# sleveque/control

Measured on AMD Instinct MI355X. Metric: Krylov iterations/s (preconditioned GMRES(10), all-at-once heat-control KKT), higher is better.
Workload: dtype f64; 1 GPU; 2-D heat control, 256^2 P1, n_t=64, beta=0.0001, T=2, BE, mode G; unknowns=8454272, krylov=gmres, left preconditioning, restart 10, classical Gram-Schmidt, parallelism=time-block rows over 1 GPU(s), transport=none, sweep_tiles=boxes from the dof coordinates (kkt_set_tile_coordinates)

## Files before the change

control_amd/csrc/capi.cpp:

```cpp
#include <algorithm>
#include <charconv>
#include <climits>
#include <cmath>
#include <cstring>
#include <string>

#include "comm.hpp"
#include "pc.hpp"
#include "relin.hpp"
#include "system.hpp"
#include "tiles.hpp"

using namespace kkt;

struct kkt_system {
    System S;
};

static std::string g_create_error;

#define KKT_TRY(h, ...)                                   \
    if (!(h)) return KKT_ERR_ARG;                         \
    System &S = (h)->S;                                   \
    try {                                                 \
// ... 15 lines not shown
    o.*F = v[0] == '1';
    return true;
}
template <int Options::*F, int LO = INT_MIN, int HI = INT_MAX>
static bool set_int(Options &o, const char *v) {
    int x = 0;
    const auto r = std::from_chars(v, v + std::strlen(v), x);
    if (r.ec != std::errc() || *r.ptr || x < LO || x > HI) return false;
    o.*F = x;
    return true;
}
static bool set_prog_mode(Options &o, const char *v) {
    static const char *names[] = {"auto", "tile", "dataflow", "flags", "w"};
    for (int k = 0; k < 5; ++k)
        if (std::strcmp(v, names[k]) == 0) {
            o.prog_mode = (ProgMode)k;
            return true;
        }
    return false;
}
static bool set_coarse_setup(Options &o, const char *v) {
    o.coarse_columns = std::strcmp(v, "columns") == 0;
    return o.coarse_columns || std::strcmp(v, "batched") == 0;
}

struct OptionKey {
    const char *key, *accepted;
    bool (*set)(Options &, const char *);
};
static const OptionKey option_keys[] = {
    {"sell_r", "1 | 2", set_int<&Options::sell_r, 1, 2>},
    {"sell_sort", "0 | 1", set_switch<&Options::sell_sort>},
    {"sell_sigma", "1..64", set_int<&Options::sell_sigma, 1, 64>},
    {"shared_rows", "0 | 1", set_switch<&Options::shared_rows>},
    {"ragged_switch", "0 | 1", set_switch<&Options::ragged_switch>},
    {"ragged_xcd", "0 | 1", set_switch<&Options::ragged_xcd>},
    {"apply_xcd", "0 | 1", set_switch<&Options::apply_xcd>},
    {"pc_xcd", "0 | 1", set_switch<&Options::pc_xcd>},
    {"interleave", "0 | 1", set_switch<&Options::interleave>},
    {"kernarg_ops", "0 | 1", set_switch<&Options::kernarg_ops>},
    {"no_graph", "0 | 1", set_switch<&Options::no_graph>},
    {"persistent", "0 | 1", set_switch<&Options::persistent>},
    {"prog_mode", "auto | tile | dataflow | flags | w", set_prog_mode},
    {"prog_waves", "1..8", set_int<&Options::prog_waves, 1, 8>},
    {"prog_steps", "0 | 1", set_switch<&Options::prog_steps>},
    {"tile_depth", "1..16", set_int<&Options::tile_depth, 1, TILE_MAX_DEPTH>},
    {"tile_waves", "1..16", set_int<&Options::tile_waves, 1, 16>},
    {"tile_unfused", "0 | 1", set_switch<&Options::tile_unfused>},
    {"tile_poll_delay", "an integer", set_int<&Options::tile_poll_delay>},
    {"lanes", "0 | 1", set_switch<&Options::lanes>},
    {"lane_chunks", "an integer", set_int<&Options::lane_chunks>},
    {"coarse_setup", "batched | columns", set_coarse_setup},
    {"coarse_keep", "0 | 1", set_switch<&Options::coarse_keep>},
    {"coarse_blocks", "0 | 1", set_switch<&Options::coarse_blocks>},
    {"coarse_rings", "0 | 1", set_switch<&Options::coarse_rings>},
    {"stage_timers", "0 | 1", set_switch<&Options::stage_timers>},
    {"verbose", "0 | 1", set_switch<&Options::verbose>},
    {"stamps", "0 | 1", set_switch<&Options::stamps>},
    {"debug_drop_handoff", "an integer", set_int<&Options::debug_drop_handoff>},
};

extern "C" {

int kkt_create(kkt_handle *out, int device_id) {
    if (!out) return KKT_ERR_ARG;
    *out = nullptr;
    try {
        int ndev = 0;
        if (hipGetDeviceCount(&ndev) != hipSuccess || ndev < 1)
            fail(KKT_ERR_HIP, "no HIP device available: libkkt has no CPU path");
        if (device_id < 0 || device_id >= ndev) fail(KKT_ERR_ARG, "device id out of range");
        HIPCHK(hipSetDevice(device_id));
        auto h = std::make_unique<kkt_system>();
        h->S.device = device_id;
        h->S.own_stream = Stream::create();
        h->S.stream = h->S.own_stream;
        *out = h.release();
        return KKT_OK;
// ... 496 lines not shown
```

control_amd/csrc/kernels.hpp:

```cpp
#pragma once
#include <hip/hip_runtime_api.h>
#include <stdint.h>

#include <string>

namespace kkt {

struct TileLaunchError {
    std::string msg;
};

constexpr int MAX_TERMS = 8;
constexpr int MDOT_MAX = 8;
constexpr int REDUCE_BLOCKS = 1024;

struct VRef {
    int64_t off;
    int32_t base;
    int32_t pad_;
};
struct Bases { const double *p[4]; };

struct SpmvTerm {
    const double *vals;
// ... 140 lines not shown
    int32_t fused_update;
    int32_t hslots;
};
bool tile_sweep_available(int W, int rpt, int threads, int hslots);
bool tile_sweep_coarse_available(int W, int rpt, int threads, int hslots);
int tile_sweep_max_hslots(int W, int rpt, int threads);
int tile_sweep_max_rpt(int W, int threads);
bool tile_sweep_fuses_update(int W, int max_terms);
size_t tile_sweep_lds_bytes(int nk_pad, int its, int coarse_nc = 0, int coarse_nslots = 0,
                            int coarse_jmax = 0, int coarse_nr_max = 0,
                            int coarse_einv_rows = 0,
                            int coarse_einv_width = 0,
                            int coarse_ring_entries = 0,
                            int coarse_jxmax = 0);
size_t tile_sweep_lds_bytes(int nk_pad, int its, const TileCoarseDev &c, int cache, bool rings);
size_t tile_sweep_lds_bytes(int nk_pad, int its, const TileCoarseDev &c);
int tile_sweep_max_tiles(int W, int rpt, int threads, size_t lds_bytes, int hslots,
                         bool coarse = false);
void launch_tile_sweep(hipStream_t s, const TileArgs &a, const TileLevel *d_levels,
                       const int32_t *d_n, const int32_t *d_grow, const uint16_t *d_lcol,
                       const int32_t *d_gpos, const uint8_t *d_rowmask, int ntiles, int threads,
                       size_t granule_words, const TileCoarseDev *h_coarse = nullptr);

void launch_csr_to_sell(hipStream_t s, const double *csr_vals, const int32_t *sell2csr,
                        double *sell_vals, int64_t n_padded);
void launch_mask_columns(hipStream_t s, double *sell_vals, const int32_t *col,
                         const uint8_t *colmask, int64_t n_padded);
void launch_vals_axpy(hipStream_t s, double *out, const double *a, double c,
                      const double *b, int64_t n_padded);
void launch_vals_differ(hipStream_t s, const double *a, const double *b, int64_t n, unsigned *flag);
void launch_vals_sym_skew(hipStream_t s, const double *a, const int32_t *tpos, double *h,
                          double *sk, int64_t n, unsigned *nonsym);
void launch_extract_dinv(hipStream_t s, const int32_t *col, const int32_t *slice_off,
                         const double *vals, const uint8_t *rowmask, double *dinv,
                         int nrows, int nslices, int R, const int32_t *perm = nullptr);

void launch_copy(hipStream_t s, double *y, const double *x, int64_t n);
void launch_fill(hipStream_t s, double *y, double v, int64_t n);
void launch_axpby(hipStream_t s, double *y, double a, const double *x, double b, int64_t n);
struct MaskJob { const uint8_t *mask; double alpha; };
void launch_mask_blocks(hipStream_t s, double *y, const double *x, const double *mx,
                        const MaskJob *d_jobs, int nblocks, int64_t nx);
void launch_time_transform_mask(hipStream_t s, double *y, const double *t, const double *xin,
                                const MaskJob *d_jobs, int kind, int n, int64_t nx,
                                const double *lo_halo, const double *hi_halo);
void launch_time_transform(hipStream_t s, double *y, const double *x, int kind, int n,
// ... 63 lines not shown
```

control_amd/csrc/pc.cpp:

```cpp
#include "pc.hpp"

#include <algorithm>
#include <chrono>
#include <cmath>
#include <cstdlib>
#include <cstdio>
#include <cstring>

namespace kkt {

static VRef vabs(const double *p) {
    return p ? VRef{(int64_t)(uintptr_t)p, 0, 0} : VRef{0, -1, 0};
}

SchurPC::SchurPC(System &S, const kkt_pc_desc &d) : S_(S), d_(d) {
    if (!S.finalized) fail(KKT_ERR_STATE, "kkt_set_pc_schur needs a finalized system");
    if (d.kind < KKT_PC_STATIONARY || d.kind > KKT_PC_INSTATIONARY_CN)
        fail(KKT_ERR_ARG, "unknown preconditioner kind");
    if (!d.m_indptr || !d.m_indices || !d.m_values) fail(KKT_ERR_ARG, "mass matrix missing");
    if (S.nx0 != S.nx1 || d.nx != S.nx0)
        fail(KKT_ERR_ARG, "built-in preconditioner needs equal spatial spaces of size nx");
    nx_ = d.nx;
    if (d.kind == KKT_PC_STATIONARY)
        n_ = 1;
// ... 23 lines not shown
        if (p_indptr_[0] != 0 || pn < 0) fail(KKT_ERR_ARG, "bad P indptr");
        p_indices_.assign(d.p_indices, d.p_indices + pn);
        p_values_.assign(d.p_values, d.p_values + pn);
        for (int64_t r = 0; r < nx_; ++r)
            if (p_indptr_[r + 1] < p_indptr_[r]) fail(KKT_ERR_ARG, "P indptr not monotone");
        for (int32_t c : p_indices_)
            if (c < 0 || c >= d.n_coarse) fail(KKT_ERR_ARG, "P column index out of range");
    }
    d_.p_indptr = d_.p_indices = nullptr;
    d_.p_values = nullptr;
    d_.m_indptr = d_.m_indices = nullptr;
    d_.m_values = nullptr;
    d_.bc_idx = nullptr;
    use_graph_ = !S_.opts.no_graph;
    use_programs_ = S_.opts.persistent;
    use_lanes_ = S_.opts.lanes;
    build();
}

void SchurPC::clear_program() {
    segments_.clear();
    program_mem_.release();
    il_cap_ = 0;
    sweep_levels_.clear();
    steps_.clear();
    n_events_ = 0;
    cur_lane_ = 0;
}

int SchurPC::emit_record(int lane) {
    PcStep s;
    s.kind = PcStep::EV_RECORD;
    s.lane = lane;
    s.ev = n_events_++;
    steps_.push_back(s);
    return s.ev;
}

void SchurPC::emit_wait(int lane, int ev) {
    PcStep s;
    s.kind = PcStep::EV_WAIT;
    s.lane = lane;
    s.ev = ev;
    steps_.push_back(s);
}

// ... 437 lines not shown
    if (coarse && !tile_sweep_fuses_update(tile_plan_.W, max_terms)) return false;
    if (tile_sweep_fuses_update(tile_plan_.W, max_terms) &&
        !(tile_plan_.W > 9 && S_.opts.tile_unfused && !coarse)) {
        tile_step(levels.data(), (int)levels.size(), (int)(e - k), true);
        return true;
    }
    for (size_t i = 0; i < run.size(); ++i) {
        const SweepLevel &lv = *run[i];
        TileLevel L = levels[i];
        size_t first_cheb = lv.first;
        if (L.n_upd > 0) {
            out.push_back(steps_[lv.first]);
            first_cheb = lv.first + 1;
            L.n_upd = 0;
            L.prev_in_lds = 0;
            L.bin = lv.b_after;
            L.bout = nullptr;
        }
        tile_step(&L, 1, (int)(lv.last - first_cheb), false);
    }
    return true;
}

void SchurPC::fuse_programs() {
    if (!use_programs_) return;
    if (!d_err_) {
        d_err_ = handle_mem_.alloc<unsigned>(64 + 16 * 1024);
        HIPCHK(hipMemset(d_err_, 0, (64 + 16 * 1024) * sizeof(unsigned)));
    }
    const bool tile_wanted = S_.opts.prog_mode == ProgMode::Auto || S_.opts.prog_mode == ProgMode::Tile;
    const bool use_tiles = tile_wanted && prepare_tiles();
    tile_epoch_cursor_ = 0;
    tile_cepoch_cursor_ = 0;
    tile_cleared_ = false;
    if (!legacy_tried_) {
        legacy_tried_ = true;
        legacy_ok_ = setup_row_programs();
    }
    if (!use_tiles && !legacy_ok_) {
        use_programs_ = false;
        return;
    }
    auto gather_out = [](const RowOp &op) -> int64_t {
        return (op.mode == EPI_LIN && op.y2.base >= 0) ? op.y2.off : op.y.off;
    };
    std::vector<PcStep> out;
    auto emit_prog = [&](size_t q0, size_t q1) {
        std::vector<RowOp> ops;
// ... 93 lines not shown
        if (s.kind == PcStep::PROG && form < 3) form = std::max(form, s.granule ? 2 : 1);
    }
    S_.info.sweep_form = form;
    S_.info.sweep_tiles = form == 3 ? tile_plan_.ntiles : 0;
    S_.info.sweep_threads = form == 3 ? tile_plan_.threads : 0;
    S_.info.sweep_depth = form == 3 ? tile_plan_.depth : 0;
    S_.info.sweep_row_slots = form == 3 ? tile_plan_.rpt : 0;
    bool rings = false;
    for (const PcStep &s : steps_)
        if (s.kind == PcStep::TILE && s.coarse) rings = h_tile_coarse_.ring_prolong != 0;
    S_.info.sweep_coarse_rings = rings ? 1 : 0;
}

void SchurPC::plain_forms(std::vector<int32_t> &out) const {
    const Pattern &P = S_.patterns[m_pat_];
    for (const PcStep &s : steps_) {
        if (s.kind == PcStep::ROWS) {
            const int form = s.rows.shared_matrix && s.rows.R == 2 ? KKT_PC_ROWS_SHARED
                             : s.rows.single                       ? KKT_PC_ROWS_KERNARG
                                                                   : KKT_PC_ROWS_PLAIN;
            out.insert(out.end(), {form, s.rows.uniform_w, s.rows.R, s.lane, s.rows.nops, 0});
        } else if (s.kind == PcStep::ROWS_IL) {
            out.insert(out.end(), {KKT_PC_ROWS_INTERLEAVED, s.il_w, 2, s.lane, s.il_groups, 0});
        } else if (s.kind == PcStep::PROG) {
            out.insert(out.end(), {KKT_PC_PROGRAM, P.uniform_w, P.R, s.lane, s.nphases,
                                   s.gmode == 2 ? 2 : s.granule ? 1 : 0});
        } else if (s.kind == PcStep::TILE) {
            out.insert(out.end(), {KKT_PC_TILE, tile_plan_.W, tile_plan_.rpt, s.lane,
                                   tile_plan_.threads, (s.fused ? 1 : 0) | (s.coarse ? 2 : 0)});
        }
    }
}

void SchurPC::debug_read(unsigned long long *out, int n) {
    if (!d_err_) return;
    HIPCHK(hipStreamSynchronize(S_.stream));
    HIPCHK(hipMemcpy(out, d_err_ + 64, (size_t)n * 8, hipMemcpyDeviceToHost));
    HIPCHK(hipMemset(d_err_ + 64, 0, (size_t)n * 8));
}

void SchurPC::time_programs(float *ms, int *launches, int64_t *phases) {
    hipStream_t st = S_.stream;
    *ms = 0.f;
    *launches = 0;
    *phases = 0;
    std::vector<std::pair<Event, Event>> evs;
// ... 33 lines not shown
    for (size_t k = 0; k < steps_.size(); ++k) {
        replay(k, k + 1);
        HIPCHK(hipEventRecord(ev[k + 1], st));
    }
    HIPCHK(hipStreamSynchronize(st));
    for (size_t k = 0; k < steps_.size(); ++k) {
        float ms = 0.f;
        HIPCHK(hipEventElapsedTime(&ms, ev[k], ev[k + 1]));
        const PcStep &s = steps_[k];
        out->total_ms += ms;
        if (s.kind == PcStep::PROG || s.kind == PcStep::TILE) {
            out->sweeps_ms += ms;
            out->sweep_launches += 1;
            out->sweep_phases += s.nphases;
        } else if (s.kind == PcStep::ROWS && s.rows.nops == 1 && n_ > 1) {
            out->sweeps_ms += ms;
            out->sweep_launches += 1;
            out->sweep_phases += 1;
        } else if (s.kind == PcStep::COMM) {
            out->comm_ms += ms;
            out->comm_steps += 1;
        } else {
            out->batched_ms += ms;
            if (s.kind == PcStep::ROWS || s.kind == PcStep::TIME || s.kind == PcStep::ROWS_IL)
                out->batched_launches += 1;
        }
    }
}

bool SchurPC::timed_out(std::string *why) {
    if (!d_err_) return false;
    unsigned e = 0;
    HIPCHK(hipMemcpyAsync(&e, d_err_, sizeof e, hipMemcpyDeviceToHost, S_.stream));
    HIPCHK(hipStreamSynchronize(S_.stream));
    if (!e) return false;
    unsigned rec[40] = {0};
    HIPCHK(hipMemcpy(rec, d_err_, sizeof rec, hipMemcpyDeviceToHost));
    HIPCHK(hipMemset(d_err_, 0, sizeof rec));
    std::string msg = "persistent sweep kernel timed out waiting for a neighbour workgroup";
    if (e & 4u)
        msg += " (tile form: tile " + std::to_string(rec[8]) + ", hand-off " +
               std::to_string(rec[9]) + ", local row " + std::to_string(rec[10]) +
               ", global row " + std::to_string(rec[11]) + ", tags seen new " +
               std::to_string(rec[12]) + "/" + std::to_string(rec[13]) + " old " +
               std::to_string(rec[14]) + "/" + std::to_string(rec[15]) +
               (rec[16] ? ", both iterates)" : ", newest iterate only)");
    if (e & 8u)
// ... 809 lines not shown
bool SchurPC::emit_solves_interleaved(const std::vector<Solve> &sv, int its, double emin,
                                      double emax) {
    if (!S_.opts.interleave || S_.opts.lanes) return false;
    const size_t m = sv.size();
    for (const Solve &q : sv)
        if (q.vals != sv[0].vals || q.dinv != sv[0].dinv) return false;
    const Pattern &P = S_.patterns[m_pat_];
    if (P.R != 2) return false;
    const int ng = (int)((m + 3) / 4);
    const size_t need = (size_t)ng * 4 * (size_t)nx_;
    if (need > il_cap_) {
        for (int k = 0; k < 3; ++k) {
            il_P_[k] = program_mem_.alloc<double>(need + 32);
            HIPCHK(hipMemsetAsync(il_P_[k], 0, (need + 32) * sizeof(double), S_.stream));
        }
        il_cap_ = need;
    }
    const double scale = 2.0 / (emax + emin);
    const double alpha = 1.0 - scale * emin, mu = 1.0 / alpha, omegaprod = 2.0 / alpha;
    double c_km1 = 1.0, c_k = mu;
    auto buf = [&](int step, int g) -> double * {
        return il_P_[(step - 1) % 3] + (size_t)g * 4 * (size_t)nx_;
    };
    for (int step = 1; step <= its; ++step) {
        double k1 = 0.0, k2 = 0.0, k3 = scale;
        if (step >= 2) {
            const double c_kp1 = 2.0 * mu * c_k - c_km1;
            const double omega = omegaprod * c_k / c_kp1;
            k1 = 1.0 - omega;
            k2 = omega;
            k3 = scale * omega;
            c_km1 = c_k;
            c_k = c_kp1;
        }
        const bool last = step == its;
        std::vector<IlOp> ops(ng);
        for (int g = 0; g < ng; ++g) {
            IlOp op{};
            op.col = P.d_col;
            op.slice_off = P.d_slice_off;
            op.perm = P.d_perm;
            op.vals = sv[0].vals;
            op.dinv = sv[0].dinv;
            op.rowmask = mask_;
            op.nrows = (int32_t)nx_;
            op.nslices = P.nslices;
            op.uniform_w = P.uniform_w;
            op.nlev = (int32_t)std::min<size_t>(4, m - (size_t)g * 4);
            for (int l = 0; l < op.nlev; ++l) {
                op.b[l] = sv[(size_t)g * 4 + l].b;
                op.out[l] = last ? sv[(size_t)g * 4 + l].out : nullptr;
            }
            op.x = step >= 2 ? buf(step - 1, g) : nullptr;
            op.pkm1 = step >= 3 ? buf(step - 2, g) : nullptr;
            op.y = last ? nullptr : buf(step, g);
            op.c1 = k1;
            op.c2 = k2;
            op.c3 = k3;
            for (int l = 0; l < 4; ++l) {
                const bool live = last && l < op.nlev;
                op.post1[l] = live ? sv[(size_t)g * 4 + l].post1 : 1.0;
                op.post2[l] = live ? sv[(size_t)g * 4 + l].post2 : 1.0;
            }
            ops[g] = op;
        }
        PcStep s;
        s.kind = PcStep::ROWS_IL;
        s.d_il = program_mem_.upload(ops.data(), ops.size());
        s.il_groups = ng;
        s.il_slices = P.nslices;
        s.il_w = P.uniform_w;
        s.lane = cur_lane_;
        steps_.push_back(s);
    }
    return true;
}

void SchurPC::emit_solves(const std::vector<Solve> &sv, int its, double emin, double emax,
                          double *const P[3], int64_t pstride, bool first_done,
                          std::vector<TileCoef> *coef_out, double eimag, const Mat *mat) {
    if (coarse_cycles_ > 0 && mat && mat->einv && sv.size() == 1 && !first_done) {
        emit_coarse_solve(nullptr, sv[0], *mat);
        return;
    }
    const size_t m = sv.size();
    if (m >= 4 && !first_done && its >= 2 && eimag == 0.0 && pstride == nx_ &&
        emit_solves_interleaved(sv, its, emin, emax))
        return;
    SweepLevel solo;
    const bool record_solo = m == 1 && !first_done && its >= 2;
    if (record_solo) {
        solo.first = steps_.size();
        coef_out = &solo.coef;
    }
    std::vector<Cheb> ops(m);
    if (its == 0) {
        for (size_t q = 0; q < m; ++q)
// ... 296 lines not shown
    if (n_events_ > 0 && !side_) side_ = Stream::create();
    while ((int)events_.size() < n_events_) events_.push_back(Event::create(false));
    for (size_t k = first; k < last; ++k) {
        const PcStep &s = steps_[k];
        hipStream_t st = s.lane == 0 ? S_.stream : side_;
        switch (s.kind) {
            case PcStep::EV_RECORD:
                HIPCHK(hipEventRecord(events_[s.ev], st));
                break;
            case PcStep::EV_WAIT:
                HIPCHK(hipStreamWaitEvent(st, events_[s.ev], 0));
                break;
            case PcStep::ROWS:
                if (s.rows.shared_matrix &&
                    launch_rowops_shared(st, s.rows.d_ops, s.rows.nops, s.rows.max_slices,
                                         s.rows.R, s.rows.uniform_w, xcd))
                    break;
                launch_rowops(st, s.rows.d_ops, s.rows.nops, s.rows.max_slices, s.rows.R, B, 1,
                              s.rows.uniform_w, s.rows.single ? &s.rows.h_op : nullptr);
                break;
            case PcStep::ROWS_IL:
                launch_rowops_il(st, s.d_il, s.il_groups, s.il_slices, s.il_w, xcd);
                break;
            case PcStep::TIME:
                launch_time_transform(st, s.y, s.x, s.tkind, s.n, s.nx, s.lo_halo, s.hi_halo);
                break;
            case PcStep::COPY:
                launch_copy(st, s.y, s.x, s.nx);
                break;
            case PcStep::COARSE:
                launch_coarse_correction(st, coarse_, s.einv, s.cr, s.x, s.y, s.nx);
                break;
            case PcStep::PROG: {
                const Pattern &P = S_.patterns[m_pat_];
                if (s.gmode == 2)
                    launch_row_program_gw(st, s.rows.d_ops, s.nphases, prog_nwg_, prog_wpw_, d_g0_,
                                          d_g1_, granule_words_, d_err_);
                else if (s.granule)
                    launch_row_program_g(st, s.rows.d_ops, s.d_lite, s.nphases, prog_nwg_, prog_wpw_,
                                         P.uniform_w, d_g0_, d_g1_, granule_words_, d_err_);
                else
                    launch_row_program(st, s.rows.d_ops, s.nphases, prog_nwg_, prog_wpw_, P.R,
                                       P.uniform_w, d_dep_, d_flags_, d_err_, prog_lowreg_);
                break;
            }
            case PcStep::TILE: {
// ... 73 lines not shown
```

control_amd/csrc/pc.hpp:

```cpp
#pragma once
#include <map>
#include <string>
#include <vector>

#include "comm.hpp"
#include "system.hpp"
#include "tiles.hpp"

namespace kkt {

struct Spectrum {
    double emin, emax;
    int steps;
};
Spectrum jacobi_spectrum(System &S, int pattern, const double *vals, const double *dinv,
                         const uint8_t *rowmask, int max_steps,
                         bool zero_mean = false);
double jacobi_skew_radius(System &S, int pattern, const double *skew_vals, const double *dinv,
                          const uint8_t *rowmask, int max_steps, int *steps_out);

struct PcStep {
    enum Kind { ROWS, TIME, COPY, COMM, PROG, TILE, EV_RECORD, EV_WAIT, COARSE, ROWS_IL } kind;
    IlOp *d_il = nullptr;
    int il_groups = 0, il_slices = 0, il_w = 0;
    const double *einv = nullptr;
    const double *cr = nullptr;
    int lane = 0;
    int ev = -1;
    RowLaunch rows;
    double *y = nullptr;
    const double *x = nullptr;
    int tkind = 0, n = 0;
    int64_t nx = 0;
    const double *lo_halo = nullptr, *hi_halo = nullptr;
    int dst = -1, src = -1;
    int nphases = 0;
    bool granule = false;
    PhaseLite *d_lite = nullptr;
    int gmode = 0;
    TileLevel *d_levels = nullptr;
    int nlevels = 0, its = 0;
    uint32_t epoch0 = 0;
    bool fused = true;
    bool clear = false;
    bool coarse = false;
// ... 182 lines not shown
    struct Cheb {
        const double *vals;
        const double *dinv, *b, *pk, *pkm1;
        double *y;
        double c1, c2, c3, post1 = 1.0, post2 = 1.0;
    };
    void build();
    void clear_program();
    const double *block_vals(int q, int i, int j) const;
    Mat schur_matrix(const double *base_vals, double c, bool solved = true);
    void emit_lin(const std::vector<Lin> &ops);
    void emit_cheb(const std::vector<Cheb> &ops);
    double *il_P_[3] = {nullptr, nullptr, nullptr};
    size_t il_cap_ = 0;
    void emit_time(double *y, const double *x, int kind, int n, const double *lo_halo = nullptr,
                   const double *hi_halo = nullptr);
    void emit_comm(const double *send, int dst, double *recv, int src);
    struct Solve {
        const double *vals, *dinv, *b;
        double *out;
        double post1 = 1.0, post2 = 1.0;
    };
    bool emit_solves_interleaved(const std::vector<Solve> &sv, int its, double emin, double emax);
    void emit_solves(const std::vector<Solve> &sv, int its, double emin, double emax,
                     double *const P[3], int64_t pstride, bool first_done = false,
                     std::vector<TileCoef> *coef_out = nullptr, double eimag = 0.0,
                     const Mat *mat = nullptr);
    void emit_update_and_solve(Lin upd, const Solve &sv, int its, double emin, double emax,
                               double eimag = 0.0, const Mat *mat = nullptr);
    void emit_coarse_solve(const Lin *upd, const Solve &sv, const Mat &F);
    const int32_t *transpose_positions();
    int32_t *d_tpos_ = nullptr;
    bool tpos_tried_ = false;
    void push_rows(std::vector<RowOp> &r);
    void build_stationary();
    void build_BE();
    void build_CN();
    void replay(size_t first, size_t last);
};

class StokesPC : public PcBase {
   public:
    StokesPC(System &outer, System &inner, System &commutator, const kkt_pc_stokes_desc &d);
    void run() override;
    double *in() override { return in_; }
    double *out() override { return out_; }
// ... 48 lines not shown
```

control_amd/csrc/system.hpp:

```cpp
#pragma once
#include <hip/hip_runtime_api.h>
#include <stdint.h>

#include <map>
#include <memory>
#include <string>
#include <tuple>
#include <vector>

#include "../../include/kkt.h"
#include "devmem.hpp"
#include "kernels.hpp"

namespace kkt {

struct Error {
    int code;
    std::string msg;
};
[[noreturn]] void fail(int code, const std::string &msg);
enum class ProgMode { Auto, Tile, Dataflow, Flags, W };
struct Options {
    int sell_r = 2, sell_sigma = 8;
    bool sell_sort = true, shared_rows = true, ragged_switch = true;
    bool ragged_xcd = true, apply_xcd = false, pc_xcd = true;
    bool interleave = true, kernarg_ops = false, no_graph = false, lanes = false;
    int lane_chunks = 4;
    bool persistent = true, prog_steps = true, tile_unfused = false;
    ProgMode prog_mode = ProgMode::Auto;
    int prog_waves = 0, tile_depth = 0, tile_waves = 0;
    bool coarse_columns = false;
    bool coarse_keep = false, coarse_blocks = true;
    bool coarse_rings = true;
    bool stage_timers = false, verbose = false, stamps = false;
    int tile_poll_delay = 24, debug_drop_handoff = 0;
};

struct Pattern {
    int64_t nrows = 0, ncols = 0, nnz = 0;
    int R = 2;
    int nslices = 0;
    int64_t nslots = 0;
    int64_t npadded = 0;
    int max_width = 0;
    int uniform_w = -1;
    uint64_t hash = 0;
    std::vector<int32_t> h_indptr, h_indices;
    int32_t *d_col = nullptr;
    int32_t *d_slice_off = nullptr;
    std::vector<int32_t> h_slice_off;
    int64_t sell_index(int64_t r, int k) const {
        const int64_t C = 64 * R, pos = pos_of(r), s = pos / C, rin = pos - s * C;
        return ((int64_t)h_slice_off[s] + k) * C + (rin % 64) * R + rin / 64;
    }
    int32_t *d_sell2csr = nullptr;
    std::vector<int32_t> h_row_of, h_pos_of;
// ... 223 lines not shown
```

control_amd/multiblock.py:

```python
from __future__ import annotations

import ctypes as C
import os
from dataclasses import dataclass
from typing import Optional, Sequence

import numpy as np

from . import _lib

__all__ = ["Nullspace", "NoneNullspace", "ConstantNullspace", "DirichletBCNullspace",
           "FullNullspace", "MultiBlockSystem", "SchurPC", "StokesPC", "KSPResult",
           "ChebSpec", "PatternOnly"]

Q00, Q01, Q10, Q11 = 0, 1, 2, 3
_KSP_TYPES = {"gmres": 0, "fgmres": 1, "minres": 2}
_PC_SIDES = {"left": 0, "right": 1, 0: 0, 1: 1}


class Nullspace:
    """``preconditioner.py:75-116`` (the corrections themselves run on the device)."""


class NoneNullspace(Nullspace):
# ... 120 lines not shown
        indptr, indices, data = A
    else:
        if not getattr(A, "has_sorted_indices", True):
            A = A.sorted_indices()
        A = A.tocsr()
        indptr, indices, data = A.indptr, A.indices, A.data
    return (np.ascontiguousarray(indptr, dtype=np.int32),
            np.ascontiguousarray(indices, dtype=np.int32),
            np.ascontiguousarray(data, dtype=np.float64))


def _array_of(v, n, nx):
    if hasattr(v, "dat") and hasattr(v.dat, "data"):
        v = v.dat.data
    a = np.asarray(v)
    if a.dtype != np.float64 or a.size != n * nx:
        raise ValueError("vector of wrong size or dtype")
    return a.reshape(n, nx)


_ENV_OPTION_KEYS = ("sell_r", "sell_sort", "no_graph", "persistent", "prog_mode", "prog_waves",
                    "prog_steps", "tile_depth", "tile_waves", "lanes", "lane_chunks",
                    "kernarg_ops", "shared_rows", "verbose", "stamps", "tile_poll_delay",
                    "tile_unfused", "stage_timers", "sell_sigma", "interleave", "coarse_rings")


class MultiBlockSystem:

    def __init__(self, space_0, space_1, block_00, block_01, block_10, block_11, *,
                 n_blocks_00=1, n_blocks_11=1, sub_n_blocks_00_0=None,
                 sub_n_blocks_11_0=None, nullspace_0=None, nullspace_1=None,
                 form_compiler_parameters=None, CN=False, device=0, comm=None, options=None,
                 share_values=True, shard_families=1):
        if nullspace_0 is None:
            nullspace_0 = tuple(NoneNullspace() for _ in range(n_blocks_00))
        if nullspace_1 is None:
            nullspace_1 = tuple(NoneNullspace() for _ in range(n_blocks_11))
        nx0, nx1 = _space_dim(space_0), _space_dim(space_1)

        def check_blocks(block, n_row_blocks, n_col_blocks):
            if len(block) != n_row_blocks * n_col_blocks:
                raise ValueError("Unexpected dimension of blocks")
        check_blocks(block_00, n_blocks_00, n_blocks_00)
        check_blocks(block_01, n_blocks_00, n_blocks_11)
        check_blocks(block_10, n_blocks_11, n_blocks_00)
        check_blocks(block_11, n_blocks_11, n_blocks_11)

# ... 379 lines not shown
```

include/kkt.h:

```cpp
#ifndef KKT_H
#define KKT_H

#include <stdint.h>

#ifdef __cplusplus
extern "C" {
#endif

typedef struct kkt_system *kkt_handle;

enum {
    KKT_OK = 0,
    KKT_ERR_ARG = -1,
    KKT_ERR_HIP = -2,
    KKT_ERR_STATE = -3,
    KKT_ERR_CALLBACK = -4,
    KKT_ERR_COMM = -5
};

enum { KKT_Q00 = 0, KKT_Q01 = 1, KKT_Q10 = 2, KKT_Q11 = 3 };

enum { KKT_KSP_GMRES = 0, KKT_KSP_FGMRES = 1, KKT_KSP_MINRES = 2 };
enum { KKT_PC_SIDE_DEFAULT = -1, KKT_PC_LEFT = 0, KKT_PC_RIGHT = 1 };

// ... 197 lines not shown
int kkt_debug_coarse_matrices(kkt_handle h, double *out, int64_t cap);
int kkt_debug_coarse_inverses(kkt_handle h, double *out, int64_t cap);
int kkt_debug_dense_inverse(kkt_handle h, int n, int nmat, const double *a, double *inv, int *bad);

enum { KKT_KRYLOV_MDOT = 0, KKT_KRYLOV_ORTHOGONALISE = 1, KKT_KRYLOV_BUILD_SOLUTION = 2,
       KKT_KRYLOV_SCALE_INV = 3, KKT_KRYLOV_AXPBY = 4, KKT_KRYLOV_COPY = 5, KKT_KRYLOV_FILL = 6,
       KKT_KRYLOV_NORM2 = 7, KKT_KRYLOV_MAXPY = 8 };
#define KKT_KRYLOV_PAD (-6.02214076e23)
int kkt_debug_krylov_op(kkt_handle h, int op, int64_t n, int nv, const double *w, const double *V,
                        const double *coef, double a, double b, double *w_out,
                        double *scalars_out, double *arena_out);

typedef struct kkt_steplock {
    int n_steps;
    int restart;
    const double *V;
    double *h;
    double *v_next;
} kkt_steplock;
int kkt_debug_set_steplock(kkt_handle h, const kkt_steplock *lock);

enum { KKT_APPLY_FORM_INTS = 4, KKT_PC_FORM_INTS = 6 };
enum { KKT_PC_ROWS_PLAIN = 0, KKT_PC_ROWS_SHARED = 1, KKT_PC_ROWS_KERNARG = 2,
       KKT_PC_ROWS_INTERLEAVED = 3, KKT_PC_PROGRAM = 4, KKT_PC_TILE = 5 };
int kkt_debug_apply_forms(kkt_handle h, int32_t *out, int cap);
int kkt_debug_pc_forms(kkt_handle h, int32_t *out, int cap);

enum { KKT_PC_SOLVE_VALS = 9, KKT_PC_MATRIX_VALS = 6 };
enum { KKT_PC_SWEEP_FIRST = 0, KKT_PC_SWEEP_SECOND = 1, KKT_PC_SWEEP_FORWARD = 2,
       KKT_PC_SWEEP_BACKWARD = 3, KKT_PC_SWEEP_KP = 4 };
enum { KKT_PC_EST_GIVEN = 0, KKT_PC_EST_LANCZOS = 1, KKT_PC_EST_SHARED = 2, KKT_PC_EST_NONE = 3,
       KKT_PC_EST_ZERO_MEAN = 4, KKT_PC_EST_UPPER = 5 };
int kkt_debug_pc_solves(kkt_handle h, double *out, int cap);
int kkt_debug_pc_matrices(kkt_handle h, double *out, int cap);

typedef struct kkt_info {
    int64_t n_local;
    int64_t n_blocks_stored;
    int64_t n_value_arrays;
    int64_t n_patterns;
    int64_t nnz_blocks;
    int64_t rows_blocks;
    int64_t bytes_algorithmic;
    int64_t bytes_device_values;
    int64_t bytes_device_index;
    int64_t bytes_streamed;
    double last_solve_ms;
// ... 30 lines not shown
```

Before: 146.3 Krylov iterations/s.

## Fuse interleaved Chebyshev mass solves into LDS-resident temporal tile kernel

Adds a tiled kernel that runs several Chebyshev steps of the batched mass-matrix solves inside one workgroup. Each tile keeps its halo-extended rows in LDS and handles four levels per group as double4. This replaces per-step interleaved row-op launches, each of which streams the whole vectors through global memory. It is enabled by default when a byte model predicts fewer bytes moved, and it adds redundant halo computation plus extra ping-pong buffers.

```diff
diff --git a/control_amd/csrc/capi.cpp b/control_amd/csrc/capi.cpp
--- a/control_amd/csrc/capi.cpp
+++ b/control_amd/csrc/capi.cpp
@@ -61,6 +61,12 @@
 static bool set_coarse_setup(Options &o, const char *v) {
     o.coarse_columns = std::strcmp(v, "columns") == 0;
     return o.coarse_columns || std::strcmp(v, "batched") == 0;
+}
+
+static bool set_mass_tile_waves(Options &o, const char *v) {
+    if (std::strcmp(v, "0") != 0 && std::strcmp(v, "4") != 0 && std::strcmp(v, "8") != 0) return false;
+    o.mass_tile_waves = v[0] - '0';
+    return true;
 }
 
 struct OptionKey {
@@ -93,6 +99,11 @@
     {"coarse_keep", "0 | 1", set_switch<&Options::coarse_keep>},
     {"coarse_blocks", "0 | 1", set_switch<&Options::coarse_blocks>},
     {"coarse_rings", "0 | 1", set_switch<&Options::coarse_rings>},
+    {"mass_tiles", "0 | 1", set_switch<&Options::mass_tiles>},
+    {"mass_tile_depth", "0..8", set_int<&Options::mass_tile_depth, 0, MASS_TILE_MAX_DEPTH>},
+    {"mass_tile_rows", "0..65536", set_int<&Options::mass_tile_rows, 0, 65536>},
+    {"mass_tile_levels", "0..4096", set_int<&Options::mass_tile_levels, 0, 4096>},
+    {"mass_tile_waves", "0 | 4 | 8", set_mass_tile_waves},
     {"stage_timers", "0 | 1", set_switch<&Options::stage_timers>},
     {"verbose", "0 | 1", set_switch<&Options::verbose>},
     {"stamps", "0 | 1", set_switch<&Options::stamps>},
diff --git a/control_amd/csrc/kernels.hpp b/control_amd/csrc/kernels.hpp
--- a/control_amd/csrc/kernels.hpp
+++ b/control_amd/csrc/kernels.hpp
@@ -186,6 +186,33 @@
                        const int32_t *d_gpos, const uint8_t *d_rowmask, int ntiles, int threads,
                        size_t granule_words, const TileCoarseDev *h_coarse = nullptr);
 
+constexpr int MASS_TILE_MAX_DEPTH = 8;
+struct MassTileGroup {
+    const double *b[4];
+    double *out[4];
+    double post1[4], post2[4];
+    int32_t nlev, pad_;
+};
+struct MassTileArgs {
+    const int32_t *n, *grow, *gpos;
+    const uint16_t *lcol;
+    const int32_t *masked;
+    const double *vals, *dinv;
+    const MassTileGroup *groups;
+    const double *in_new, *in_old;
+    double *out_new, *out_old;
+    int64_t nx;
+    int32_t nmasked, ngroups, nk_pad, W;
+    int32_t s0, k, last, pad_;
+    double coef[MASS_TILE_MAX_DEPTH][3];
+};
+int mass_tile_kernel_width(int W);
+int mass_tile_max_rpt(int threads);
+size_t mass_tile_lds_bytes(int nk_pad);
+int mass_tile_prepare(int W, int rpt, int threads, size_t lds_bytes);
+void launch_mass_tile(hipStream_t s, const MassTileArgs &a, int ntiles, int grid_y, int rpt,
+                      int threads);
+
 void launch_csr_to_sell(hipStream_t s, const double *csr_vals, const int32_t *sell2csr,
                         double *sell_vals, int64_t n_padded);
 void launch_mask_columns(hipStream_t s, double *sell_vals, const int32_t *col,
diff --git a/control_amd/csrc/mass_tile_kernels.hip b/control_amd/csrc/mass_tile_kernels.hip
--- /dev/null
+++ b/control_amd/csrc/mass_tile_kernels.hip
@@ -0,0 +1,219 @@
+#include "kernels.hpp"
+
+#include <hip/hip_runtime.h>
+
+namespace kkt {
+
+#define KKT_GLOBAL __attribute__((address_space(1)))
+typedef KKT_GLOBAL const double *gcd_p;
+typedef KKT_GLOBAL double *gd_p;
+typedef KKT_GLOBAL const int32_t *gci_p;
+typedef KKT_GLOBAL const uint16_t *gcu16_p;
+typedef double d4 __attribute__((ext_vector_type(4)));
+typedef KKT_GLOBAL const d4 *gcd4_p;
+typedef KKT_GLOBAL d4 *gd4_p;
+
+__device__ __forceinline__ void lds_barrier_mt() {
+    asm volatile("s_waitcnt lgkmcnt(0)\n\ts_barrier" ::: "memory");
+}
+
+template <int W, int RPT, int T>
+__global__ __launch_bounds__(T) void pc_tile_cheb(const MassTileArgs A) {
+    extern __shared__ d4 X4[];
+    __shared__ int sn[TILE_DEPTH_MAX + 1];
+    const int tid = threadIdx.x, tile = blockIdx.x;
+    const int nkp = A.nk_pad, k = A.k;
+    const gci_p nt = (gci_p)A.n + (size_t)tile * (TILE_DEPTH_MAX + 1);
+    if (tid <= TILE_DEPTH_MAX) sn[tid] = nt[tid];
+    const int n0 = nt[0], nk = nt[k], nk1 = nt[k - 1];
+    const d4 zero4 = d4{0.0, 0.0, 0.0, 0.0};
+    if (tid == 0) {
+        X4[nkp - 1] = zero4;
+        X4[2 * (size_t)nkp - 1] = zero4;
+    }
+    const gci_p grow = (gci_p)A.grow + (size_t)tile * nkp;
+    double v[RPT][W], dinv[RPT];
+    int col[RPT][W], gr[RPT];
+    {
+        const int PW = A.W;
+        const gcu16_p lcol = (gcu16_p)A.lcol + (size_t)tile * RPT * PW * T + tid;
+        const gci_p gpos = (gci_p)A.gpos + (size_t)tile * RPT * PW * T + tid;
+        const gcd_p vals = (gcd_p)A.vals, dv = (gcd_p)A.dinv;
+#pragma unroll
+        for (int sl = 0; sl < RPT; ++sl) {
+            const int r = sl * T + tid;
+#pragma unroll
+            for (int e = 0; e < W; ++e) {
+                col[sl][e] = e < PW ? lcol[(size_t)(sl * PW + e) * T] : 0;
+                const int gp = e < PW ? gpos[(size_t)(sl * PW + e) * T] : -1;
+                v[sl][e] = gp >= 0 ? vals[gp] : 0.0;
+            }
+            gr[sl] = r < nk1 ? grow[r] : -1;
+            dinv[sl] = gr[sl] >= 0 ? dv[gr[sl]] : 0.0;
+        }
+    }
+    const int64_t nx = A.nx;
+    const bool first = A.s0 == 0, last = A.last != 0;
+    for (int g = blockIdx.y; g < A.ngroups; g += gridDim.y) {
+        const MassTileGroup &G = A.groups[g];
+        const int nlev = G.nlev;
+        int cur = 0;
+        {
+            d4 *Xc = X4, *Xo = X4 + nkp;
+            if (first) {
+                for (int l = tid; l < nk; l += T) {
+                    Xc[l] = zero4;
+                    Xo[l] = zero4;
+                }
+            } else {
+                const gcd4_p pn = (gcd4_p)A.in_new + (size_t)g * nx;
+                const gcd4_p po = (gcd4_p)A.in_old + (size_t)g * nx;
+                const bool has_old = A.s0 >= 2;
+                for (int l = tid; l < nk; l += T) {
+                    const int gl = grow[l];
+                    Xc[l] = pn[gl];
+                    Xo[l] = has_old ? po[gl] : zero4;
+                }
+            }
+        }
+        d4 b[RPT];
+#pragma unroll
+        for (int sl = 0; sl < RPT; ++sl) {
+            double bb[4];
+#pragma unroll
+            for (int l = 0; l < 4; ++l)
+                bb[l] = (gr[sl] >= 0 && l < nlev) ? ((gcd_p)G.b[l])[gr[sl]] : 0.0;
+            b[sl] = d4{bb[0], bb[1], bb[2], bb[3]};
+        }
+        __syncthreads();
+        for (int j = 1; j <= k; ++j) {
+            const int s = A.s0 + j;
+            const int nv = sn[k - j];
+            const bool has_new = s >= 2, has_old = s >= 3, fin = last && j == k;
+            const double c1 = A.coef[j - 1][0], c2 = A.coef[j - 1][1], c3 = A.coef[j - 1][2];
+            d4 q1 = d4{1.0, 1.0, 1.0, 1.0}, q2 = q1;
+            if (fin) {
+                q1 = d4{G.post1[0], G.post1[1], G.post1[2], G.post1[3]};
+                q2 = d4{G.post2[0], G.post2[1], G.post2[2], G.post2[3]};
+            }
+            const d4 *Xc = X4 + (size_t)cur * nkp;
+            d4 *Xo = X4 + (size_t)(cur ^ 1) * nkp;
+#pragma unroll
+            for (int sl = 0; sl < RPT; ++sl) {
+                if (sl * T + (tid & ~63) >= nv) continue;
+                const int r = sl * T + tid;
+                d4 acc = zero4;
+                if (has_new) {
+                    d4 xv[W];
+#pragma unroll
+                    for (int e = 0; e < W; ++e) xv[e] = Xc[col[sl][e]];
+#pragma unroll
+                    for (int e = 0; e < W; ++e) {
+                        acc.x = __builtin_fma(v[sl][e], xv[e].x, acc.x);
+                        acc.y = __builtin_fma(v[sl][e], xv[e].y, acc.y);
+                        acc.z = __builtin_fma(v[sl][e], xv[e].z, acc.z);
+                        acc.w = __builtin_fma(v[sl][e], xv[e].w, acc.w);
+                    }
+                }
+                if (r < nv) {
+                    const d4 e0 = Xo[r], e1 = Xc[r];
+                    const double a_[4] = {acc.x, acc.y, acc.z, acc.w};
+                    const double p0_[4] = {e0.x, e0.y, e0.z, e0.w}, p1_[4] = {e1.x, e1.y, e1.z, e1.w};
+                    const double b_[4] = {b[sl].x, b[sl].y, b[sl].z, b[sl].w};
+                    const double f1[4] = {q1.x, q1.y, q1.z, q1.w}, f2[4] = {q2.x, q2.y, q2.z, q2.w};
+                    double o[4];
+#pragma unroll
+                    for (int l = 0; l < 4; ++l) {
+                        double t = has_old ? c1 * p0_[l] : 0.0;
+                        if (has_new) t += c2 * p1_[l];
+                        t += c3 * (dinv[sl] * (b_[l] - a_[l]));
+                        o[l] = f2[l] * (f1[l] * t);
+                    }
+                    Xo[r] = d4{o[0], o[1], o[2], o[3]};
+                }
+            }
+            lds_barrier_mt();
+            cur ^= 1;
+        }
+        {
+            const d4 *Xc = X4 + (size_t)cur * nkp, *Xo = X4 + (size_t)(cur ^ 1) * nkp;
+            if (last) {
+                for (int l = tid; l < n0; l += T) {
+                    const int gl = grow[l];
+                    const d4 x = Xc[l];
+                    const double o[4] = {x.x, x.y, x.z, x.w};
+#pragma unroll
+                    for (int q = 0; q < 4; ++q)
+                        if (q < nlev) ((gd_p)G.out[q])[gl] = o[q];
+                }
+                if (tile == 0) {
+                    const gci_p mr = (gci_p)A.masked;
+                    for (int i = tid; i < A.nmasked; i += T) {
+                        const int gl = mr[i];
+#pragma unroll
+                        for (int q = 0; q < 4; ++q)
+                            if (q < nlev) ((gd_p)G.out[q])[gl] = 0.0;
+                    }
+                }
+            } else {
+                const gd4_p pn = (gd4_p)A.out_new + (size_t)g * nx;
+                const gd4_p po = (gd4_p)A.out_old + (size_t)g * nx;
+                for (int l = tid; l < n0; l += T) {
+                    const int gl = grow[l];
+                    pn[gl] = Xc[l];
+                    po[gl] = Xo[l];
+                }
+            }
+        }
+        __syncthreads();
+    }
+}
+
+typedef void (*mass_tile_fn)(const MassTileArgs);
+
+static mass_tile_fn pick_mass_tile(int W, int rpt, int threads) {
+#define KKT_MT(w, r, t) \
+    if (W == w && rpt == r && threads == t) return pc_tile_cheb<w, r, t>;
+#define KKT_MTW(w)                                                                             \
+    KKT_MT(w, 1, 256) KKT_MT(w, 2, 256) KKT_MT(w, 3, 256) KKT_MT(w, 4, 256) KKT_MT(w, 1, 512) \
+    KKT_MT(w, 2, 512) KKT_MT(w, 3, 512)
+    KKT_MTW(5)
+    KKT_MTW(7)
+    KKT_MTW(9)
+#undef KKT_MTW
+#undef KKT_MT
+    return nullptr;
+}
+
+int mass_tile_kernel_width(int W) { return W < 1 ? 0 : W <= 5 ? 5 : W <= 7 ? 7 : W <= 9 ? 9 : 0; }
+
+int mass_tile_max_rpt(int threads) { return threads == 256 ? 4 : threads == 512 ? 3 : 0; }
+
+size_t mass_tile_lds_bytes(int nk_pad) { return 2 * (size_t)nk_pad * sizeof(d4); }
+
+int mass_tile_prepare(int W, int rpt, int threads, size_t lds_bytes) {
+    const mass_tile_fn f = pick_mass_tile(mass_tile_kernel_width(W), rpt, threads);
+    constexpr int LDS_LIMIT = 160 * 1024 - 1024;
+    if (!f || lds_bytes > (size_t)LDS_LIMIT) return 0;
+    if (hipFuncSetAttribute((const void *)f, hipFuncAttributeMaxDynamicSharedMemorySize,
+                            LDS_LIMIT) != hipSuccess)
+        return 0;
+    int per_cu = 0;
+    if (hipOccupancyMaxActiveBlocksPerMultiprocessor(&per_cu, f, threads, lds_bytes) != hipSuccess)
+        return 0;
+    return per_cu;
+}
+
+void launch_mass_tile(hipStream_t s, const MassTileArgs &a, int ntiles, int grid_y, int rpt,
+                      int threads) {
+    if (ntiles <= 0 || grid_y <= 0 || a.ngroups <= 0) return;
+    const mass_tile_fn f = pick_mass_tile(mass_tile_kernel_width(a.W), rpt, threads);
+    if (!f) throw TileLaunchError{"mass tile kernel: no variant for this plan"};
+    (void)hipGetLastError();
+    hipLaunchKernelGGL(f, dim3(ntiles, grid_y), dim3(threads), mass_tile_lds_bytes(a.nk_pad), s, a);
+    const hipError_t e = hipGetLastError();
+    if (e != hipSuccess)
+        throw TileLaunchError{std::string("mass tile kernel: launch: ") + hipGetErrorString(e)};
+}
+
+}
diff --git a/control_amd/csrc/pc.cpp b/control_amd/csrc/pc.cpp
--- a/control_amd/csrc/pc.cpp
+++ b/control_amd/csrc/pc.cpp
@@ -69,6 +69,9 @@
     segments_.clear();
     program_mem_.release();
     il_cap_ = 0;
+    mt_cap_ = 0;
+    mass_solves_.clear();
+    mass_launches_.clear();
     sweep_levels_.clear();
     steps_.clear();
     n_events_ = 0;
@@ -552,8 +555,177 @@
     return true;
 }
 
+bool SchurPC::prepare_mass_tiles() {
+    if (mass_tried_) return mass_ok_;
+    mass_tried_ = true;
+    const Pattern &P = S_.patterns[m_pat_];
+    if (P.R != 2 || mass_tile_kernel_width(P.max_width) == 0) return false;
+    int dev_id = 0;
+    if (hipGetDevice(&dev_id) != hipSuccess ||
+        hipDeviceGetAttribute(&mass_cus_, hipDeviceAttributeMultiprocessorCount, dev_id) != hipSuccess ||
+        mass_cus_ < 1)
+        return false;
+    std::vector<uint8_t> hmask;
+    if (!bc_idx_.empty()) {
+        hmask.assign(P.nrows, 0);
+        for (int32_t k : bc_idx_) hmask[k] = 1;
+    }
+    int64_t live = 0;
+    for (int64_t r = 0; r < P.nrows; ++r) live += hmask.empty() || !hmask[r];
+    if (live < 1) return false;
+    const double *tc = (S_.tile_dim > 0 && (int64_t)S_.tile_coords.size() == P.nrows * S_.tile_dim)
+                           ? S_.tile_coords.data() : nullptr;
+    const bool chosen = S_.opts.mass_tile_depth > 0 || S_.opts.mass_tile_rows > 0;
+    const int K = S_.opts.mass_tile_depth > 0 ? S_.opts.mass_tile_depth : 5;
+    const int rows = S_.opts.mass_tile_rows > 0 ? S_.opts.mass_tile_rows : 512;
+    const int ntiles = (int)std::max<int64_t>(1, (live + rows - 1) / rows);
+    auto any_halo = [](int, int, int) { return 1 << 20; };
+    bool ok = false;
+    for (int threads : {256, 512}) {
+        if (S_.opts.mass_tile_waves && threads != 64 * S_.opts.mass_tile_waves) continue;
+        if (build_tile_plan(P, ntiles, K, threads, mass_tile_max_rpt(threads), mass_plan_,
+                            hmask.empty() ? nullptr : hmask.data(), 0, tc, S_.tile_dim, any_halo)) {
+            ok = true;
+            break;
+        }
+    }
+    if (!ok) return false;
+    const TilePlan &tp = mass_plan_;
+    const size_t lds = mass_tile_lds_bytes(tp.nk_pad);
+    mass_per_cu_ = mass_tile_prepare(tp.W, tp.rpt, tp.threads, lds);
+    if (mass_per_cu_ < 1) return false;
+    double tile_bytes = 0.0, plain_bytes = 0.0;
+    for (int t = 0; t < tp.ntiles; ++t) {
+        const int32_t *nt = &tp.n[(size_t)t * (TILE_MAX_DEPTH + 1)];
+        tile_bytes += 64.0 * nt[K] + 32.0 * nt[K - 1] + 64.0 * nt[0];
+        plain_bytes += 160.0 * K * nt[0];
+    }
+    const double ratio = tile_bytes / std::max(1.0, plain_bytes);
+    const bool pays = ratio < 0.6;
+    if (S_.opts.verbose)
+        std::fprintf(stderr, "[kkt] mass tile form: %d tiles x %d threads, K %d, W %d, %d row slots; "
+                     "largest tile: %lld own rows, %lld computed rows; redundancy %.2f; %zu bytes of "
+                     "LDS, %d workgroups per CU; modelled bytes %.2f of the plain steps'%s\n",
+                     tp.ntiles, tp.threads, K, tp.W, tp.rpt, (long long)tp.max_own,
+                     (long long)tp.max_rows, tp.mean_redundancy, lds, mass_per_cu_, ratio,
+                     pays || chosen ? "" : ": off");
+    if (!pays && !chosen) return false;
+    mass_plan_.upload(handle_mem_);
+    if (!bc_idx_.empty()) d_masked_ = handle_mem_.upload(bc_idx_.data(), bc_idx_.size());
+    mass_ok_ = true;
+    return true;
+}
+
+void SchurPC::fuse_mass_tiles() {
+    if (!S_.opts.mass_tiles || S_.opts.lanes || mass_solves_.empty()) return;
+    bool any = false;
+    for (const MassSolve &ms : mass_solves_) any = any || ms.its >= 2;
+    if (!any || !prepare_mass_tiles()) return;
+    const TilePlan &tp = mass_plan_;
+    const int K = tp.depth;
+    std::vector<PcStep> out;
+    std::vector<size_t> new_index(steps_.size() + 1, 0);
+    size_t k = 0, q = 0;
+    while (k < steps_.size()) {
+        while (q < mass_solves_.size() && mass_solves_[q].first < k) ++q;
+        const MassSolve *ms = q < mass_solves_.size() && mass_solves_[q].first == k ? &mass_solves_[q] : nullptr;
+        bool run = ms && ms->its >= 2 && k + ms->its <= steps_.size();
+        for (int i = 0; run && i < ms->its; ++i) run = steps_[k + i].kind == PcStep::ROWS_IL;
+        if (!run) {
+            new_index[k] = out.size();
+            out.push_back(steps_[k++]);
+            continue;
+        }
+        const size_t m = ms->sv.size();
+        const int ng = (int)((m + 3) / 4);
+        const size_t need = (size_t)ng * 4 * (size_t)nx_;
+        if (need > mt_cap_) {
+            for (int i = 0; i < 4; ++i) {
+                mt_P_[i] = program_mem_.alloc<double>(need + 32);
+                HIPCHK(hipMemsetAsync(mt_P_[i], 0, (need + 32) * sizeof(double), S_.stream));
+            }
+            mt_cap_ = need;
+        }
+        std::vector<MassTileGroup> groups(ng);
+        for (int g = 0; g < ng; ++g) {
+            MassTileGroup G{};
+            G.nlev = (int32_t)std::min<size_t>(4, m - (size_t)g * 4);
+            for (int l = 0; l < 4; ++l) {
+                const bool live = l < G.nlev;
+                const Solve *sv = live ? &ms->sv[(size_t)g * 4 + l] : nullptr;
+                G.b[l] = live ? sv->b : nullptr;
+                G.out[l] = live ? sv->out : nullptr;
+                G.post1[l] = live ? sv->post1 : 1.0;
+                G.post2[l] = live ? sv->post2 : 1.0;
+            }
+            groups[g] = G;
+        }
+        const MassTileGroup *d_groups = program_mem_.upload(groups.data(), groups.size());
+        int gpw = S_.opts.mass_tile_levels > 0 ? (S_.opts.mass_tile_levels + 3) / 4 : 0;
+        if (gpw <= 0) {
+            const int64_t slots = (int64_t)mass_per_cu_ * mass_cus_;
+            const int gy = (int)std::max<int64_t>(1, std::min<int64_t>(ng, slots / tp.ntiles));
+            gpw = (ng + gy - 1) / gy;
+        }
+        const int grid_y = (ng + gpw - 1) / gpw;
+        const int nl = (ms->its + K - 1) / K;
+        for (int i = 0; i < ms->its; ++i) new_index[k + i] = out.size();
+        for (int j = 0; j < nl; ++j) {
+            MassLaunch ml;
+            MassTileArgs &a = ml.a;
+            a = MassTileArgs{};
+            a.n = tp.d_n;
+            a.grow = tp.d_grow;
+            a.gpos = tp.d_gpos;
+            a.lcol = tp.d_lcol;
+            a.masked = d_masked_;
+            a.nmasked = (int32_t)bc_idx_.size();
+            a.vals = ms->sv[0].vals;
+            a.dinv = ms->sv[0].dinv;
+            a.groups = d_groups;
+            const int wr = j & 1, rd = wr ^ 1;
+            a.in_new = mt_P_[2 * rd];
+            a.in_old = mt_P_[2 * rd + 1];
+            a.out_new = mt_P_[2 * wr];
+            a.out_old = mt_P_[2 * wr + 1];
+            a.nx = nx_;
+            a.ngroups = ng;
+            a.nk_pad = tp.nk_pad;
+            a.W = tp.W;
+            a.s0 = j * K;
+            a.k = std::min(K, ms->its - a.s0);
+            a.last = j + 1 == nl ? 1 : 0;
+            for (int i = 0; i < a.k; ++i) {
+                const TileCoef &c = ms->coef[a.s0 + i];
+                a.coef[i][0] = c.c1;
+                a.coef[i][1] = c.c2;
+                a.coef[i][2] = c.c3;
+            }
+            ml.grid_y = grid_y;
+            PcStep s;
+            s.kind = PcStep::TILE_CHEB;
+            s.mt = (int)mass_launches_.size();
+            s.lane = steps_[k].lane;
+            mass_launches_.push_back(ml);
+            out.push_back(s);
+        }
+        if (S_.opts.verbose)
+            std::fprintf(stderr, "[kkt] mass tile form: a solve of %d steps on %zu levels as %d "
+                         "launches of %d x %d workgroups (%d level groups each)\n", ms->its, m, nl,
+                         tp.ntiles, grid_y, gpw);
+        k += ms->its;
+    }
+    new_index[steps_.size()] = out.size();
+    for (SweepLevel &lv : sweep_levels_) {
+        lv.first = new_index[lv.first];
+        lv.last = new_index[lv.last];
+    }
+    steps_.swap(out);
+}
+
 void SchurPC::fuse_programs() {
     if (!use_programs_) return;
+    fuse_mass_tiles();
     if (!d_err_) {
         d_err_ = handle_mem_.alloc<unsigned>(64 + 16 * 1024);
         HIPCHK(hipMemset(d_err_, 0, (64 + 16 * 1024) * sizeof(unsigned)));
@@ -693,6 +865,9 @@
             out.insert(out.end(), {form, s.rows.uniform_w, s.rows.R, s.lane, s.rows.nops, 0});
         } else if (s.kind == PcStep::ROWS_IL) {
             out.insert(out.end(), {KKT_PC_ROWS_INTERLEAVED, s.il_w, 2, s.lane, s.il_groups, 0});
+        } else if (s.kind == PcStep::TILE_CHEB) {
+            out.insert(out.end(), {KKT_PC_TILE_CHEB, mass_plan_.W, mass_plan_.rpt, s.lane,
+                                   mass_launches_[s.mt].a.k, mass_plan_.threads});
         } else if (s.kind == PcStep::PROG) {
             out.insert(out.end(), {KKT_PC_PROGRAM, P.uniform_w, P.R, s.lane, s.nphases,
                                    s.gmode == 2 ? 2 : s.granule ? 1 : 0});
@@ -772,7 +947,8 @@
             out->comm_steps += 1;
         } else {
             out->batched_ms += ms;
-            if (s.kind == PcStep::ROWS || s.kind == PcStep::TIME || s.kind == PcStep::ROWS_IL)
+            if (s.kind == PcStep::ROWS || s.kind == PcStep::TIME || s.kind == PcStep::ROWS_IL ||
+                s.kind == PcStep::TILE_CHEB)
                 out->batched_launches += 1;
         }
     }
@@ -1628,6 +1804,10 @@
     auto buf = [&](int step, int g) -> double * {
         return il_P_[(step - 1) % 3] + (size_t)g * 4 * (size_t)nx_;
     };
+    MassSolve rec;
+    rec.first = steps_.size();
+    rec.its = its;
+    rec.sv = sv;
     for (int step = 1; step <= its; ++step) {
         double k1 = 0.0, k2 = 0.0, k3 = scale;
         if (step >= 2) {
@@ -1639,6 +1819,7 @@
             c_km1 = c_k;
             c_k = c_kp1;
         }
+        rec.coef.push_back(TileCoef{k1, k2, k3});
         const bool last = step == its;
         std::vector<IlOp> ops(ng);
         for (int g = 0; g < ng; ++g) {
@@ -1679,6 +1860,7 @@
         s.lane = cur_lane_;
         steps_.push_back(s);
     }
+    mass_solves_.push_back(std::move(rec));
     return true;
 }
 
@@ -2021,6 +2203,16 @@
             case PcStep::ROWS_IL:
                 launch_rowops_il(st, s.d_il, s.il_groups, s.il_slices, s.il_w, xcd);
                 break;
+            case PcStep::TILE_CHEB: {
+                const MassLaunch &ml = mass_launches_[s.mt];
+                try {
+                    launch_mass_tile(st, ml.a, mass_plan_.ntiles, ml.grid_y, mass_plan_.rpt,
+                                     mass_plan_.threads);
+                } catch (const TileLaunchError &e) {
+                    fail(KKT_ERR_HIP, e.msg);
+                }
+                break;
+            }
             case PcStep::TIME:
                 launch_time_transform(st, s.y, s.x, s.tkind, s.n, s.nx, s.lo_halo, s.hi_halo);
                 break;
diff --git a/control_amd/csrc/pc.hpp b/control_amd/csrc/pc.hpp
--- a/control_amd/csrc/pc.hpp
+++ b/control_amd/csrc/pc.hpp
@@ -20,7 +20,8 @@
                           const uint8_t *rowmask, int max_steps, int *steps_out);
 
 struct PcStep {
-    enum Kind { ROWS, TIME, COPY, COMM, PROG, TILE, EV_RECORD, EV_WAIT, COARSE, ROWS_IL } kind;
+    enum Kind { ROWS, TIME, COPY, COMM, PROG, TILE, EV_RECORD, EV_WAIT, COARSE, ROWS_IL, TILE_CHEB } kind;
+    int mt = -1;
     IlOp *d_il = nullptr;
     int il_groups = 0, il_slices = 0, il_w = 0;
     const double *einv = nullptr;
@@ -249,6 +250,26 @@
         double post1 = 1.0, post2 = 1.0;
     };
     bool emit_solves_interleaved(const std::vector<Solve> &sv, int its, double emin, double emax);
+    struct MassSolve {
+        size_t first = 0;
+        int its = 0;
+        std::vector<Solve> sv;
+        std::vector<TileCoef> coef;
+    };
+    std::vector<MassSolve> mass_solves_;
+    struct MassLaunch {
+        MassTileArgs a;
+        int grid_y = 1;
+    };
+    std::vector<MassLaunch> mass_launches_;
+    TilePlan mass_plan_;
+    bool mass_tried_ = false, mass_ok_ = false;
+    int mass_per_cu_ = 0, mass_cus_ = 0;
+    int32_t *d_masked_ = nullptr;
+    double *mt_P_[4] = {nullptr, nullptr, nullptr, nullptr};
+    size_t mt_cap_ = 0;
+    bool prepare_mass_tiles();
+    void fuse_mass_tiles();
     void emit_solves(const std::vector<Solve> &sv, int its, double emin, double emax,
                      double *const P[3], int64_t pstride, bool first_done = false,
                      std::vector<TileCoef> *coef_out = nullptr, double eimag = 0.0,
diff --git a/control_amd/csrc/system.hpp b/control_amd/csrc/system.hpp
--- a/control_amd/csrc/system.hpp
+++ b/control_amd/csrc/system.hpp
@@ -32,6 +32,8 @@
     bool coarse_columns = false;
     bool coarse_keep = false, coarse_blocks = true;
     bool coarse_rings = true;
+    bool mass_tiles = true;
+    int mass_tile_depth = 0, mass_tile_rows = 0, mass_tile_levels = 0, mass_tile_waves = 0;
     bool stage_timers = false, verbose = false, stamps = false;
     int tile_poll_delay = 24, debug_drop_handoff = 0;
 };
diff --git a/control_amd/multiblock.py b/control_amd/multiblock.py
--- a/control_amd/multiblock.py
+++ b/control_amd/multiblock.py
@@ -166,7 +166,9 @@
 _ENV_OPTION_KEYS = ("sell_r", "sell_sort", "no_graph", "persistent", "prog_mode", "prog_waves",
                     "prog_steps", "tile_depth", "tile_waves", "lanes", "lane_chunks",
                     "kernarg_ops", "shared_rows", "verbose", "stamps", "tile_poll_delay",
-                    "tile_unfused", "stage_timers", "sell_sigma", "interleave", "coarse_rings")
+                    "tile_unfused", "stage_timers", "sell_sigma", "interleave", "coarse_rings",
+                    "mass_tiles", "mass_tile_depth", "mass_tile_rows", "mass_tile_levels",
+                    "mass_tile_waves")
 
 
 class MultiBlockSystem:
diff --git a/include/kkt.h b/include/kkt.h
--- a/include/kkt.h
+++ b/include/kkt.h
@@ -243,7 +243,7 @@
 
 enum { KKT_APPLY_FORM_INTS = 4, KKT_PC_FORM_INTS = 6 };
 enum { KKT_PC_ROWS_PLAIN = 0, KKT_PC_ROWS_SHARED = 1, KKT_PC_ROWS_KERNARG = 2,
-       KKT_PC_ROWS_INTERLEAVED = 3, KKT_PC_PROGRAM = 4, KKT_PC_TILE = 5 };
+       KKT_PC_ROWS_INTERLEAVED = 3, KKT_PC_PROGRAM = 4, KKT_PC_TILE = 5, KKT_PC_TILE_CHEB = 6 };
 int kkt_debug_apply_forms(kkt_handle h, int32_t *out, int cap);
 int kkt_debug_pc_forms(kkt_handle h, int32_t *out, int cap);
 
```

Measured after the change: 153.3 Krylov iterations/s (median of 6 runs). +4.8%, better.
